# alibaba/TePDist

Hardware: AMD Instinct MI355X
Metric: tokens/sec (higher is better)
Workload: dtype bf16; 1 GPU; model=gpt2-345m, global_batch=64, seq_len=1024, parallelism=auto-planned-graph:dp1tp1pp1mesh[]micro1

## Files before the change

### tepdist_amd/ops/csrc/bindings.cpp

```cpp

#include <pybind11/pybind11.h>

#include <hip/hip_runtime.h>

#include <stdexcept>
#include <string>

#include "common.h"
#include "gemm_plan.h"
#include "kernels.h"

namespace py = pybind11;
using namespace tepdist;

namespace {

hipStream_t S(uintptr_t s) { return reinterpret_cast<hipStream_t>(s); }

void check_launch() { HIP_CHECK(hipGetLastError()); }

}

PYBIND11_MODULE(_tepdist_hip, m) {
  m.doc() = "TePDist-AMD gfx950 kernel library";

  m.def("gemm", [](uintptr_t A, uintptr_t B, uintptr_t C, uintptr_t Cpre,
                   uintptr_t bias, int M, int N, int K, int lda, int ldb,
                   int ldc, int64_t sa, int64_t sb, int64_t sc, int batch,
                   bool a_kc, bool b_kc, int epi, uintptr_t splitk_ws,
                   uintptr_t stream, uintptr_t colsum_out) {
    gemm_bf16(reinterpret_cast<void*>(A), reinterpret_cast<void*>(B),
              reinterpret_cast<void*>(C), reinterpret_cast<void*>(Cpre),
              reinterpret_cast<void*>(bias), M, N, K, lda, ldb, ldc, sa, sb,
              sc, batch, a_kc, b_kc, epi, reinterpret_cast<float*>(splitk_ws),
              reinterpret_cast<void*>(colsum_out), S(stream));
    check_launch();
  }, py::arg("A"), py::arg("B"), py::arg("C"), py::arg("Cpre"),
     py::arg("bias"), py::arg("M"), py::arg("N"), py::arg("K"),
     py::arg("lda"), py::arg("ldb"), py::arg("ldc"), py::arg("sa"),
     py::arg("sb"), py::arg("sc"), py::arg("batch"), py::arg("a_kc"),
     py::arg("b_kc"), py::arg("epi"), py::arg("splitk_ws"),
     py::arg("stream"), py::arg("colsum_out") = 0);

  m.def("gemm_ws_floats", [](int M, int N, int K, int lda, int ldb,
                             bool a_kc, bool b_kc, int epi, int batch,
                             bool colsum) {
    const GemmPlan p = gemm_plan(M, N, K, lda, ldb, a_kc, b_kc, epi, batch);
    if (colsum)
      if (const char* why = colsum_why_not(p, a_kc, b_kc, batch))
        throw std::runtime_error(std::string("gemm_ws_floats: ") + why);
    return gemm_ws_floats(p, M, N, colsum);
  }, py::arg("M"), py::arg("N"), py::arg("K"), py::arg("lda"),
     py::arg("ldb"), py::arg("a_kc") = true, py::arg("b_kc") = true,
     py::arg("epi") = 0, py::arg("batch") = 1, py::arg("colsum") = false);

  m.def("gemm_plan", [](int M, int N, int K, int lda, int ldb, bool a_kc,
                        bool b_kc, int epi, int batch) {
    const GemmPlan p = gemm_plan(M, N, K, lda, ldb, a_kc, b_kc, epi, batch);
    return py::make_tuple(p.kernel, p.split_k, p.k_chunk,
                          p.why_not ? p.why_not : "");
  }, py::arg("M"), py::arg("N"), py::arg("K"), py::arg("lda"),
     py::arg("ldb"), py::arg("a_kc") = true, py::arg("b_kc") = true,
     py::arg("epi") = 0, py::arg("batch") = 1);

  m.def("transpose", [](uintptr_t in, uintptr_t out, int R, int C,
                        int64_t si, int64_t so, int batch,
                        uintptr_t stream) {
    transpose_bf16(reinterpret_cast<void*>(in), reinterpret_cast<void*>(out),
                   R, C, si, so, batch, S(stream));
    check_launch();
  });

  m.def("layernorm_fwd", [](uintptr_t x, uintptr_t g, uintptr_t b, uintptr_t y,
                            uintptr_t mean, uintptr_t rstd, int rows, int cols,
                            float eps, uintptr_t stream, uintptr_t res,
                            uintptr_t sum_out) {
    layernorm_fwd_bf16(reinterpret_cast<void*>(x), reinterpret_cast<void*>(g),
                       reinterpret_cast<void*>(b), reinterpret_cast<void*>(y),
                       reinterpret_cast<float*>(mean),
                       reinterpret_cast<float*>(rstd), rows, cols, eps,
                       S(stream), reinterpret_cast<void*>(res),
                       reinterpret_cast<void*>(sum_out));
    check_launch();
  }, pybind11::arg("x"), pybind11::arg("g"), pybind11::arg("b"),
     pybind11::arg("y"), pybind11::arg("mean"), pybind11::arg("rstd"),
     pybind11::arg("rows"), pybind11::arg("cols"), pybind11::arg("eps"),
     pybind11::arg("stream"), pybind11::arg("res") = 0,
     pybind11::arg("sum_out") = 0);

  m.def("layernorm_bwd", [](uintptr_t dy, uintptr_t x, uintptr_t g,
                            uintptr_t mean, uintptr_t rstd, uintptr_t dx,
                            uintptr_t dg_part, uintptr_t db_part,
                            uintptr_t dgamma, uintptr_t dbeta, int rows,
                            int cols, int part_rows, uintptr_t stream,
                            uintptr_t dsum) {
    layernorm_bwd_bf16(reinterpret_cast<void*>(dy), reinterpret_cast<void*>(x),
                       reinterpret_cast<void*>(g),
                       reinterpret_cast<float*>(mean),
                       reinterpret_cast<float*>(rstd),
                       reinterpret_cast<void*>(dx),
                       reinterpret_cast<float*>(dg_part),
                       reinterpret_cast<float*>(db_part), rows, cols,
                       part_rows, S(stream), reinterpret_cast<void*>(dsum));
    check_launch();
    layernorm_bwd_reduce(reinterpret_cast<float*>(dg_part),
                         reinterpret_cast<float*>(db_part),
                         reinterpret_cast<void*>(dgamma),
                         reinterpret_cast<void*>(dbeta), part_rows, cols,
                         S(stream));
    check_launch();
  }, pybind11::arg("dy"), pybind11::arg("x"), pybind11::arg("g"),
     pybind11::arg("mean"), pybind11::arg("rstd"), pybind11::arg("dx"),
     pybind11::arg("dg_part"), pybind11::arg("db_part"),
     pybind11::arg("dgamma"), pybind11::arg("dbeta"), pybind11::arg("rows"),
     pybind11::arg("cols"), pybind11::arg("part_rows"),
     pybind11::arg("stream"), pybind11::arg("dsum") = 0);

  m.def("softmax_fwd", [](uintptr_t x, uintptr_t p, int64_t rows, int cols,
                          int sq, float scale, bool causal, uintptr_t stream) {
    softmax_fwd_bf16(reinterpret_cast<void*>(x), reinterpret_cast<void*>(p),
                     rows, cols, sq, scale, causal, S(stream));
    check_launch();
  });

  m.def("softmax_bwd", [](uintptr_t dp, uintptr_t p, uintptr_t ds,
                          int64_t rows, int cols, float scale,
                          uintptr_t stream) {
    softmax_bwd_bf16(reinterpret_cast<void*>(dp), reinterpret_cast<void*>(p),
                     reinterpret_cast<void*>(ds), rows, cols, scale,
                     S(stream));
    check_launch();
  });

  m.def("attention_fwd", [](uintptr_t q, uintptr_t k, uintptr_t v,
                            uintptr_t o, uintptr_t lse, int B, int H,
                            int seq, int D, float scale, bool causal,
                            int64_t q_bs, int64_t q_hs, int64_t q_rs,
                            int64_t o_bs, int64_t o_hs, int64_t o_rs,
                            uintptr_t stream) {
    attention_fwd_bf16(reinterpret_cast<void*>(q), reinterpret_cast<void*>(k),
                       reinterpret_cast<void*>(v), reinterpret_cast<void*>(o),
                       reinterpret_cast<float*>(lse), B, H, seq, D, scale,
                       causal, q_bs, q_hs, q_rs, o_bs, o_hs, o_rs, S(stream));
    check_launch();
  });

  m.def("attention_bwd", [](uintptr_t q, uintptr_t k, uintptr_t v,
                            uintptr_t o, uintptr_t dout, uintptr_t lse,
                            uintptr_t delta, uintptr_t dq, uintptr_t dk,
                            uintptr_t dv, int B, int H, int seq, int D,
                            float scale, bool causal, int64_t q_bs,
                            int64_t q_hs, int64_t q_rs, int64_t o_bs,
                            int64_t o_hs, int64_t o_rs, uintptr_t stream) {
    attention_bwd_bf16(
        reinterpret_cast<void*>(q), reinterpret_cast<void*>(k),
        reinterpret_cast<void*>(v), reinterpret_cast<void*>(o),
        reinterpret_cast<void*>(dout), reinterpret_cast<float*>(lse),
        reinterpret_cast<float*>(delta), reinterpret_cast<void*>(dq),
        reinterpret_cast<void*>(dk), reinterpret_cast<void*>(dv), B, H, seq,
        D, scale, causal, q_bs, q_hs, q_rs, o_bs, o_hs, o_rs, S(stream));
    check_launch();
  });

  m.def("decode_attention", [](uintptr_t q, uintptr_t k_new, uintptr_t v_new,
                               uintptr_t k_cache, uintptr_t v_cache,
                               uintptr_t pos, int pos_stride, uintptr_t out,
                               uintptr_t ws, int B, int H, int Hkv,
                               int S_max, int D, float scale, int splits,
                               bool rope, float rope_theta, int64_t q_bs,
                               int64_t q_hs, int64_t n_bs, int64_t n_hs,
                               int64_t c_bs, int64_t c_hs, int64_t c_rs,
                               uintptr_t stream) {
    decode_attention_bf16(
        reinterpret_cast<void*>(q), reinterpret_cast<void*>(k_new),
        reinterpret_cast<void*>(v_new), reinterpret_cast<void*>(k_cache),
        reinterpret_cast<void*>(v_cache),
        reinterpret_cast<const int64_t*>(pos), pos_stride,
        reinterpret_cast<void*>(out), reinterpret_cast<float*>(ws), B, H,
        Hkv, S_max, D, scale, splits, rope, rope_theta, q_bs, q_hs, n_bs,
        n_hs, c_bs, c_hs, c_rs, S(stream));
    check_launch();
  });

  m.def("moe_route_ws_ints", &moe_route_ws_ints);

  m.def("moe_route", [](uintptr_t gates, bool gates_fp32, uintptr_t topi,
                        uintptr_t slot, uintptr_t src, uintptr_t counts,
                        uintptr_t ws, int T, int E, int k, int C,
                        uintptr_t stream) {
    moe_route(reinterpret_cast<const void*>(gates), gates_fp32,
              reinterpret_cast<int*>(topi), reinterpret_cast<int*>(slot),
              reinterpret_cast<int*>(src), reinterpret_cast<int*>(counts),
              reinterpret_cast<int*>(ws), T, E, k, C, S(stream));
    check_launch();
  });

  m.def("moe_gather_rows", [](uintptr_t in, uintptr_t src, uintptr_t w,
                              uintptr_t out, int T, int k, int64_t EC, int d,
                              uintptr_t stream) {
    moe_gather_rows_bf16(reinterpret_cast<const void*>(in),
                         reinterpret_cast<const int*>(src),
                         reinterpret_cast<const float*>(w),
                         reinterpret_cast<void*>(out), T, k, EC, d,
                         S(stream));
    check_launch();
  });

  m.def("moe_reduce_rows", [](uintptr_t in, uintptr_t slot, uintptr_t w,
                              uintptr_t out, int T, int k, int64_t EC, int d,
                              uintptr_t stream) {
    moe_reduce_rows_bf16(reinterpret_cast<const void*>(in),
                         reinterpret_cast<const int*>(slot),
                         reinterpret_cast<const float*>(w),
                         reinterpret_cast<void*>(out), T, k, EC, d,
                         S(stream));
    check_launch();
  });

  m.def("moe_combine_dw", [](uintptr_t y, uintptr_t dout, uintptr_t slot,
                             uintptr_t dw, int T, int k, int64_t EC, int d,
                             uintptr_t stream) {
    moe_combine_dw_bf16(reinterpret_cast<const void*>(y),
                        reinterpret_cast<const void*>(dout),
                        reinterpret_cast<const int*>(slot),
                        reinterpret_cast<float*>(dw), T, k, EC, d, S(stream));
    check_launch();
  });

  m.def("embedding_fwd",[](uintptr_t ids, uintptr_t table, uintptr_t out,
                            int64_t n_ids, int dim, uintptr_t stream) {
    embedding_fwd_bf16(reinterpret_cast<const int64_t*>(ids),
                       reinterpret_cast<void*>(table),
                       reinterpret_cast<void*>(out), n_ids, dim, S(stream));
    check_launch();
  });

  m.def("embedding_bwd", [](uintptr_t dy, uintptr_t ids, uintptr_t grad_f32,
                            uintptr_t grad_bf16, int64_t n_ids, int vocab,
                            int dim, uintptr_t stream) {
    embedding_bwd_bf16(reinterpret_cast<void*>(dy),
                       reinterpret_cast<const int64_t*>(ids),
// ... 165 lines not shown
```

### tepdist_amd/ops/csrc/kernels.h

```cpp
#pragma once

#include <hip/hip_runtime.h>
#include <hip/hip_bf16.h>
#include <cstdint>

namespace tepdist {

using bf16 = __hip_bfloat16;

void gemm_bf16(const void* A, const void* B, void* C, void* c_pre,
               const void* bias, int M, int N, int K, int lda, int ldb,
               int ldc, int64_t stride_a, int64_t stride_b, int64_t stride_c,
               int batch, bool a_kc, bool b_kc, int epi, float* splitk_ws,
               void* colsum_out, hipStream_t stream);
void gemm256_bf16(const void* A, const void* B, void* C, void* c_pre,
                  const void* bias, int M, int N, int K, int lda, int ldb,
                  int ldc, int64_t stride_a, int64_t stride_b,
                  int64_t stride_c, int batch, bool k_outer, int epi,
                  int split_k, int k_chunk, float* colsum_parts,
                  hipStream_t stream);

void transpose_bf16(const void* in, void* out, int R, int C,
                    int64_t stride_in, int64_t stride_out, int batch,
                    hipStream_t stream);
void cast_ws_f32_bf16(const float* ws, void* db_out, int cols,
                      hipStream_t stream);
void transpose_dy_bf16(const void* dy, const void* pre, void* dy_t,
                       void* dy_nat, float* bias_ws, int R, int C,
                       hipStream_t stream);

void layernorm_fwd_bf16(const void* x, const void* gamma, const void* beta,
                        void* y, float* mean, float* rstd, int rows, int cols,
                        float eps, hipStream_t stream,
                        const void* res = nullptr, void* sum_out = nullptr);
void layernorm_bwd_bf16(const void* dy, const void* x, const void* gamma,
                        const float* mean, const float* rstd, void* dx,
                        float* dgamma_part, float* dbeta_part, int rows,
                        int cols, int part_rows, hipStream_t stream,
                        const void* dsum = nullptr);
void layernorm_bwd_reduce(const float* dgamma_part, const float* dbeta_part,
                          void* dgamma, void* dbeta, int part_rows, int cols,
                          hipStream_t stream);

void softmax_fwd_bf16(const void* x, void* p, int64_t rows, int cols, int sq,
                      float scale, bool causal, hipStream_t stream);
void softmax_bwd_bf16(const void* dp, const void* p, void* ds, int64_t rows,
                      int cols, float scale, hipStream_t stream);

void attention_fwd_bf16(const void* q, const void* k, const void* v, void* o,
                        float* lse, int B, int H, int S, int D, float scale,
                        bool causal, int64_t q_bs, int64_t q_hs, int64_t q_rs,
                        int64_t o_bs, int64_t o_hs, int64_t o_rs,
                        hipStream_t stream);
void attention_bwd_bf16(const void* q, const void* k, const void* v,
                        const void* o, const void* dout, const float* lse,
                        float* delta, void* dq, void* dk, void* dv,
                        int B, int H, int S, int D, float scale, bool causal,
                        int64_t q_bs, int64_t q_hs, int64_t q_rs,
                        int64_t o_bs, int64_t o_hs, int64_t o_rs,
                        hipStream_t stream);

void decode_attention_bf16(const void* q, const void* k_new,
                           const void* v_new, void* k_cache, void* v_cache,
                           const int64_t* pos, int pos_stride, void* out,
                           float* ws, int B, int H, int Hkv, int S_max,
                           int D, float scale, int splits, bool rope,
                           float rope_theta, int64_t q_bs,
                           int64_t q_hs, int64_t n_bs, int64_t n_hs,
                           int64_t c_bs, int64_t c_hs, int64_t c_rs,
                           hipStream_t stream);

int64_t moe_route_ws_ints(int T, int E);
void moe_route(const void* gates, bool gates_fp32, int* topi, int* slot,
               int* src, int* counts, int* ws, int T, int E, int k, int C,
               hipStream_t stream);
void moe_gather_rows_bf16(const void* in, const int* src, const float* w,
                          void* out, int T, int k, int64_t EC, int d,
                          hipStream_t stream);
void moe_reduce_rows_bf16(const void* in, const int* slot, const float* w,
                          void* out, int T, int k, int64_t EC, int d,
                          hipStream_t stream);
void moe_combine_dw_bf16(const void* y, const void* dout, const int* slot,
                         float* dw, int T, int k, int64_t EC, int d,
                         hipStream_t stream);

void embedding_fwd_bf16(const int64_t* ids, const void* table, void* out,
                        int64_t n_ids, int dim, hipStream_t stream);
void embedding_bwd_bf16(const void* dy, const int64_t* ids, float* grad_f32,
                        void* grad_bf16, int64_t n_ids, int vocab, int dim,
                        hipStream_t stream);

void cross_entropy_fwd_bf16(const void* logits, const int64_t* targets,
                            float* nll, float* lse, int64_t rows, int cols,
                            int ignore_index, hipStream_t stream);
void cross_entropy_bwd_bf16(const void* logits, const int64_t* targets,
                            const float* lse, const float* dscale,
                            void* dlogits, int64_t rows, int cols,
                            int ignore_index, hipStream_t stream);

void dropout_fwd_bf16(const void* x, void* y, uint8_t* mask, int64_t n,
                      float p, uint64_t seed, uint64_t offset,
                      hipStream_t stream);
void dropout_bwd_bf16(const void* dy, const uint8_t* mask, void* dx, int64_t n,
                      float p, hipStream_t stream);

void gelu_fwd_bf16(const void* x, void* y, int64_t n, hipStream_t stream);
void gelu_bwd_bf16(const void* dy, const void* x, void* dx, int64_t n,
                   hipStream_t stream);
void bias_sum_bf16(const void* dy, void* db, float* ws_zeroed, int64_t rows,
                   int cols, hipStream_t stream);

void adamw_bf16(void* param, float* master, const void* grad_bf16,
                const float* grad_f32, float* exp_avg, float* exp_avg_sq,
                int64_t n, float lr, float beta1, float beta2, float eps,
                float weight_decay, float bc1, float bc2, hipStream_t stream);

void adamw_mt_bf16(const int64_t* tabs, const int64_t* numel,
                   const float* wds, const unsigned char* ptypes,
                   const int* chunks, int nchunks, int nt,
                   float lr, float beta1, float beta2, float eps, float bc1,
                   float bc2, const float* hyper, hipStream_t stream);

void tr16_probe(float* out_pattern, float* out_uniform, hipStream_t stream);
void tr16_frag_probe(int* out, int C, hipStream_t stream);

void rmsnorm_fwd_bf16(const void* x, const void* g, void* y, float* rstd,
                      int64_t rows, int cols, float eps, hipStream_t stream);
void rmsnorm_bwd_bf16(const void* dy, const void* x, const void* g,
                      const float* rstd, void* dx, void* dgamma,
                      float* dg_part, int part_rows, int64_t rows, int cols,
                      hipStream_t stream);
void rope_bf16(const void* x, void* y, int64_t tokens, int heads, int D,
               int seq_len, float theta, bool backward, hipStream_t stream);
void swiglu_fwd_bf16(const void* a, const void* b, void* y, int64_t n,
                     hipStream_t stream);
void swiglu_bwd_bf16(const void* dy, const void* a, const void* b, void* da,
                     void* db, int64_t n, hipStream_t stream);

}
```

### tepdist_amd/ops/csrc/layernorm.hip

```cpp

#include <algorithm>
#include <stdexcept>

#include "common.h"
#include "kernels.h"

namespace tepdist {

namespace {

constexpr int NT = 256;

template <int NV, bool ADD = false>
__launch_bounds__(NT) __global__
void ln_fwd_kernel(const bf16_t* __restrict__ x, const bf16_t* __restrict__ g,
                   const bf16_t* __restrict__ b, bf16_t* __restrict__ y,
                   float* __restrict__ mean_out, float* __restrict__ rstd_out,
                   int rows, int cols, float eps,
                   const bf16_t* __restrict__ res = nullptr,
                   bf16_t* __restrict__ sum_out = nullptr) {
  const int lane = threadIdx.x & 63;
  const int wid = threadIdx.x >> 6;
  const int nwaves = gridDim.x * (NT / WAVE);

  for (int row = blockIdx.x * (NT / WAVE) + wid; row < rows; row += nwaves) {
    const bf16_t* xr = x + (int64_t)row * cols;
    const bf16_t* rr = ADD ? res + (int64_t)row * cols : nullptr;
    bf16_t* sr = ADD ? sum_out + (int64_t)row * cols : nullptr;
    float vals[NV * 8];
    float s = 0.f;
#pragma unroll
    for (int v = 0; v < NV; ++v) {
      const int c0 = v * WAVE * 8 + lane * 8;
      bf16x8 xv = {};
      bf16x8 rv = {};
      if (c0 + 8 <= cols) {
        xv = *reinterpret_cast<const bf16x8*>(xr + c0);
        if (ADD) rv = *reinterpret_cast<const bf16x8*>(rr + c0);
      } else {
#pragma unroll
        for (int e = 0; e < 8; ++e)
          if (c0 + e < cols) {
            xv[e] = xr[c0 + e];
            if (ADD) rv[e] = rr[c0 + e];
          }
      }
      bf16x8 sv;
#pragma unroll
      for (int e = 0; e < 8; ++e) {
        float f = bf2f(xv[e]);
        if (ADD) {
          sv[e] = f2bf(f + bf2f(rv[e]));
          f = bf2f(sv[e]);
        }
        vals[v * 8 + e] = f;
        s += f;
      }
      if (ADD && c0 < cols) {
        if (c0 + 8 <= cols) {
          *reinterpret_cast<bf16x8*>(sr + c0) = sv;
        } else {
          for (int e = 0; e < 8 && c0 + e < cols; ++e) sr[c0 + e] = sv[e];
        }
      }
    }
    s = wave_allreduce_sum(s);
    const float mean = s / cols;
    float ss = 0.f;
#pragma unroll
    for (int v = 0; v < NV; ++v)
#pragma unroll
      for (int e = 0; e < 8; ++e) {
        const int c = v * WAVE * 8 + lane * 8 + e;
        const float d = (c < cols) ? (vals[v * 8 + e] - mean) : 0.f;
        ss += d * d;
      }
    ss = wave_allreduce_sum(ss);
    const float rstd = rsqrtf(ss / cols + eps);
    if (lane == 0) {
      mean_out[row] = mean;
      rstd_out[row] = rstd;
    }
    bf16_t* yr = y + (int64_t)row * cols;
#pragma unroll
    for (int v = 0; v < NV; ++v) {
      const int c0 = v * WAVE * 8 + lane * 8;
      if (c0 >= cols) continue;
      bf16x8 yv = {};
      if (c0 + 8 <= cols) {
        const bf16x8 gv = *reinterpret_cast<const bf16x8*>(g + c0);
        const bf16x8 bv = *reinterpret_cast<const bf16x8*>(b + c0);
#pragma unroll
        for (int e = 0; e < 8; ++e) {
          const float xhat = (vals[v * 8 + e] - mean) * rstd;
          yv[e] = f2bf(xhat * bf2f(gv[e]) + bf2f(bv[e]));
        }
        *reinterpret_cast<bf16x8*>(yr + c0) = yv;
      } else {
        for (int e = 0; e < 8 && c0 + e < cols; ++e) {
          const float xhat = (vals[v * 8 + e] - mean) * rstd;
          yr[c0 + e] = f2bf(xhat * bf2f(g[c0 + e]) + bf2f(b[c0 + e]));
        }
      }
    }
  }
}

template <int NV, bool DS = false>
__launch_bounds__(NT) __global__
void ln_bwd_kernel(const bf16_t* __restrict__ dy, const bf16_t* __restrict__ x,
                   const bf16_t* __restrict__ g, const float* __restrict__ mean,
                   const float* __restrict__ rstd, bf16_t* __restrict__ dx,
                   float* __restrict__ dg_part, float* __restrict__ db_part,
                   int rows, int cols,
                   const bf16_t* __restrict__ dsum = nullptr) {
  const int lane = threadIdx.x & 63;
  const int wid = threadIdx.x >> 6;
  const int gwave = blockIdx.x * (NT / WAVE) + wid;
  const int nwaves = gridDim.x * (NT / WAVE);

  float dg_acc[NV * 8] = {};
  float db_acc[NV * 8] = {};

  bf16x8 gvv[NV];
#pragma unroll
  for (int v = 0; v < NV; ++v) {
    const int c0 = v * WAVE * 8 + lane * 8;
    bf16x8 gv = {};
    if (c0 + 8 <= cols) {
      gv = *reinterpret_cast<const bf16x8*>(g + c0);
    } else {
      for (int e = 0; e < 8 && c0 + e < cols; ++e) gv[e] = g[c0 + e];
    }
    gvv[v] = gv;
  }

  for (int row = gwave; row < rows; row += nwaves) {
    const bf16_t* dyr = dy + (int64_t)row * cols;
    const bf16_t* xr = x + (int64_t)row * cols;
    const float mu = mean[row], rs = rstd[row];
    float c1 = 0.f, c2 = 0.f;
    bf16x8 dyvv[NV], xvv[NV];
#pragma unroll
    for (int v = 0; v < NV; ++v) {
      const int c0 = v * WAVE * 8 + lane * 8;
      bf16x8 dyv = {}, xv = {};
      if (c0 + 8 <= cols) {
        dyv = *reinterpret_cast<const bf16x8*>(dyr + c0);
        xv = *reinterpret_cast<const bf16x8*>(xr + c0);
      } else {
        for (int e = 0; e < 8 && c0 + e < cols; ++e) {
          dyv[e] = dyr[c0 + e];
          xv[e] = xr[c0 + e];
        }
      }
      dyvv[v] = dyv;
      xvv[v] = xv;
#pragma unroll
      for (int e = 0; e < 8; ++e) {
        const int c = c0 + e;
        const float d = bf2f(dyv[e]);
        const float xhat = (c < cols) ? (bf2f(xv[e]) - mu) * rs : 0.f;
        const float gg = (c < cols) ? d * bf2f(gvv[v][e]) : 0.f;
        dg_acc[v * 8 + e] += d * xhat;
        db_acc[v * 8 + e] += d;
        c1 += gg;
        c2 += gg * xhat;
      }
    }
    c1 = wave_allreduce_sum(c1) / cols;
    c2 = wave_allreduce_sum(c2) / cols;
    bf16_t* dxr = dx + (int64_t)row * cols;
    const bf16_t* dsr = DS ? dsum + (int64_t)row * cols : nullptr;
#pragma unroll
    for (int v = 0; v < NV; ++v) {
      const int c0 = v * WAVE * 8 + lane * 8;
      if (c0 >= cols) continue;
      bf16x8 dsv = {};
      if (DS) {
        if (c0 + 8 <= cols) {
          dsv = *reinterpret_cast<const bf16x8*>(dsr + c0);
        } else {
          for (int e = 0; e < 8 && c0 + e < cols; ++e) dsv[e] = dsr[c0 + e];
        }
      }
      bf16x8 dxv;
#pragma unroll
      for (int e = 0; e < 8; ++e) {
        const float xhat = (bf2f(xvv[v][e]) - mu) * rs;
        const float gg = bf2f(dyvv[v][e]) * bf2f(gvv[v][e]);
        float d = (gg - c1 - xhat * c2) * rs;
        if (DS) d += bf2f(dsv[e]);
        dxv[e] = f2bf(d);
      }
      if (c0 + 8 <= cols) {
        *reinterpret_cast<bf16x8*>(dxr + c0) = dxv;
      } else {
        for (int e = 0; e < 8 && c0 + e < cols; ++e) dxr[c0 + e] = dxv[e];
      }
    }
  }

  float* dgp = dg_part + (int64_t)gwave * cols;
  float* dbp = db_part + (int64_t)gwave * cols;
#pragma unroll
  for (int v = 0; v < NV; ++v)
#pragma unroll
    for (int e = 0; e < 8; ++e) {
      const int c = v * WAVE * 8 + lane * 8 + e;
      if (c < cols) {
        dgp[c] = dg_acc[v * 8 + e];
        dbp[c] = db_acc[v * 8 + e];
      }
    }
}

__global__ void ln_bwd_reduce_kernel(const float* __restrict__ dg_part,
                                     const float* __restrict__ db_part,
                                     bf16_t* __restrict__ dgamma,
                                     bf16_t* __restrict__ dbeta,
                                     int part_rows, int cols) {
  const int lane = threadIdx.x & 63;
  const int c = blockIdx.x * (NT / WAVE) + (threadIdx.x >> 6);
  if (c >= cols) return;
  float sg = 0.f, sb = 0.f;
  for (int r = lane; r < part_rows; r += WAVE) {
    sg += dg_part[(int64_t)r * cols + c];
    sb += db_part[(int64_t)r * cols + c];
  }
  sg = wave_allreduce_sum(sg);
  sb = wave_allreduce_sum(sb);
  if (lane == 0) {
    dgamma[c] = f2bf(sg);
    dbeta[c] = f2bf(sb);
  }
}

int nv_for(int cols) { return (cols + WAVE * 8 - 1) / (WAVE * 8); }

}

void layernorm_fwd_bf16(const void* x, const void* gamma, const void* beta,
                        void* y, float* mean, float* rstd, int rows, int cols,
                        float eps, hipStream_t stream, const void* res,
                        void* sum_out) {
  const int blocks = std::min((rows + 3) / 4, 2048);
  const dim3 g(blocks), blk(NT);
  const bf16_t* xp = static_cast<const bf16_t*>(x);
  const bf16_t* gp = static_cast<const bf16_t*>(gamma);
  const bf16_t* bp = static_cast<const bf16_t*>(beta);
  bf16_t* yp = static_cast<bf16_t*>(y);
  const bf16_t* rp = static_cast<const bf16_t*>(res);
  bf16_t* sp = static_cast<bf16_t*>(sum_out);
#define LN_FWD(NV)                                                           \
  do {                                                                       \
    if (rp)                                                                  \
      hipLaunchKernelGGL((ln_fwd_kernel<NV, true>), g, blk, 0, stream, xp,  \
                         gp, bp, yp, mean, rstd, rows, cols, eps, rp, sp);  \
    else                                                                     \
      hipLaunchKernelGGL((ln_fwd_kernel<NV, false>), g, blk, 0, stream, xp, \
                         gp, bp, yp, mean, rstd, rows, cols, eps);          \
  } while (0)
  switch (nv_for(cols)) {
    case 1: LN_FWD(1); break;
    case 2: LN_FWD(2); break;
    case 3: LN_FWD(3); break;
    case 4: LN_FWD(4); break;
    case 5: LN_FWD(5); break;
    case 6: LN_FWD(6); break;
    default: throw std::runtime_error("layernorm: cols > 3072 unsupported");
  }
#undef LN_FWD
}

void layernorm_bwd_bf16(const void* dy, const void* x, const void* gamma,
                        const float* mean, const float* rstd, void* dx,
                        float* dgamma_part, float* dbeta_part, int rows,
                        int cols, int part_rows, hipStream_t stream,
                        const void* dsum) {
  const int blocks = part_rows / (NT / WAVE);
  const dim3 g(blocks), blk(NT);
  const bf16_t* dyp = static_cast<const bf16_t*>(dy);
  const bf16_t* xp = static_cast<const bf16_t*>(x);
  const bf16_t* gp = static_cast<const bf16_t*>(gamma);
  bf16_t* dxp = static_cast<bf16_t*>(dx);
  const bf16_t* dsp = static_cast<const bf16_t*>(dsum);
#define LN_BWD(NV)                                                           \
  do {                                                                       \
    if (dsp)                                                                 \
      hipLaunchKernelGGL((ln_bwd_kernel<NV, true>), g, blk, 0, stream, dyp, \
                         xp, gp, mean, rstd, dxp, dgamma_part, dbeta_part,  \
                         rows, cols, dsp);                                  \
    else                                                                     \
      hipLaunchKernelGGL((ln_bwd_kernel<NV, false>), g, blk, 0, stream,     \
                         dyp, xp, gp, mean, rstd, dxp, dgamma_part,         \
                         dbeta_part, rows, cols);                          \
  } while (0)
  switch (nv_for(cols)) {
    case 1: LN_BWD(1); break;
    case 2: LN_BWD(2); break;
    case 3: LN_BWD(3); break;
    case 4: LN_BWD(4); break;
    case 5: LN_BWD(5); break;
    case 6: LN_BWD(6); break;
    default: throw std::runtime_error("layernorm: cols > 3072 unsupported");
  }
#undef LN_BWD
}

void layernorm_bwd_reduce(const float* dgamma_part, const float* dbeta_part,
                          void* dgamma, void* dbeta, int part_rows, int cols,
                          hipStream_t stream) {
  hipLaunchKernelGGL(ln_bwd_reduce_kernel, dim3((cols + 3) / 4), dim3(NT),
                     0, stream, dgamma_part, dbeta_part,
                     static_cast<bf16_t*>(dgamma), static_cast<bf16_t*>(dbeta),
                     part_rows, cols);
}

}
```

### tepdist_amd/ops/hip.py

```python

from __future__ import annotations

import math
import os
from typing import Optional, Tuple

import torch

try:
    from tepdist_amd.ops import _tepdist_hip as ext
except ImportError as e:
    raise ImportError(
        "tepdist_amd HIP extension not built. Run "
        "`python tepdist_amd/ops/build_ext.py` (hipcc cross-compiles on a "
        "GPU-less box). No eager fallback is provided on GPU.") from e

BF16 = torch.bfloat16


def _stream() -> int:
    return torch.cuda.current_stream().cuda_stream


def _p(t: Optional[torch.Tensor]) -> int:
# ... 242 lines not shown
                  _stream())
    return out


def _wgrad_in_place(dyl: torch.Tensor, x: torch.Tensor) -> bool:
    (M, N), K = dyl.shape, x.shape[1]
    return dyl.stride(-1) == 1 and x.stride(-1) == 1 and ext.gemm_plan(
        N, K, M, dyl.stride(0), x.stride(0), False, False, 0, 1)[0] == 256


def wgrad(dyl: torch.Tensor, x: torch.Tensor, has_bias: bool):
    M, N = dyl.shape
    K = x.shape[1]
    def _db():
        return _bias_sum(dyl.contiguous()) if has_bias else None

    if not _wgrad_in_place(dyl, x):
        return matmul(dyl.t(), x), _db()

    def _hand():
        db = torch.empty(N, dtype=BF16, device=dyl.device) \
            if has_bias else None
        dw = _gemm_raw(dyl, x, False, False, N, K, M, dyl.stride(0),
                       x.stride(0), 0, 0, 1, colsum_out=db)[0]
        return dw, db

    def _lib():
        return torch.matmul(dyl.t(), x), _db()

    return _pick_backend(("lin_bw", M, N, K, has_bias), _hand, _lib)()


def linear_bwd(dy: torch.Tensor, x: torch.Tensor, w: torch.Tensor,
               has_bias: bool, act: str, pre_act: Optional[torch.Tensor]):
    dy = dy.contiguous()
    M, N = dy.shape
    K = w.shape[1]

    if _wgrad_in_place(dy, x):
        if act == "gelu":
            dyl = torch.empty_like(dy)
            ext.gelu_bwd(dy.data_ptr(), pre_act.data_ptr(), dyl.data_ptr(),
                         dy.numel(), _stream())
        else:
            dyl = dy

        def _dx_hip():
            wT = transpose2d(w)
            return _gemm_raw(dyl, wT, True, True, M, K, N, N, N, 0, 0, 1)[0]

        dx = _pick_backend(("lin_bx", M, N, K), _dx_hip,
                           lambda: torch.matmul(dyl, w))()
        dw, db = wgrad(dyl, x, has_bias)
        return dx, dw, db

    def _hip():
        dyl = dy
        wT = transpose2d(w)
        dyT = torch.empty(N, M, dtype=BF16, device=dy.device)
        if act == "gelu":
            dy_eff = torch.empty_like(dyl)
            ext.transpose_dy(dyl.data_ptr(), pre_act.data_ptr(),
                             dyT.data_ptr(), dy_eff.data_ptr(), 0, M, N,
                             _stream())
            dyl = dy_eff
        else:
            ext.transpose_dy(dyl.data_ptr(), 0, dyT.data_ptr(), 0, 0, M, N,
                             _stream())
        xT = transpose2d(x)
        dx, _ = _gemm_raw(dyl, wT, True, True, M, K, N, N, N, 0, 0, 1)
        dw, _ = _gemm_raw(dyT, xT, True, True, N, K, M, M, M, 0, 0, 1)
        return dx, dw, dyl

    def _blt():
        if act == "gelu":
            dyl = torch.empty_like(dy)
            ext.gelu_bwd(dy.data_ptr(), pre_act.data_ptr(), dyl.data_ptr(),
                         dy.numel(), _stream())
        else:
            dyl = dy
        dx = torch.matmul(dyl, w)
        dw = torch.matmul(dyl.t(), x)
        return dx, dw, dyl

    fn = _pick_backend(("lin_b", M, N, K, act), _hip, _blt)
    dx, dw, dy_eff = fn()
    db = None
    if has_bias:
        db = _bias_sum(dy_eff)
    return dx, dw, db


def matmul(a: torch.Tensor, b: torch.Tensor) -> torch.Tensor:
    key = ("mm", tuple(a.shape), tuple(b.shape),
           a.stride(-1) == 1, b.stride(-1) == 1)
    return _pick_backend(key, lambda: _matmul_hip(a, b),
                         lambda: torch.matmul(a, b))()


def _matmul_hip(a: torch.Tensor, b: torch.Tensor) -> torch.Tensor:
    assert a.dtype == BF16 and b.dtype == BF16
    squeeze = a.dim() == 2 and b.dim() == 2
    lead_shape = (a if a.dim() >= b.dim() else b).shape[:-2]
    if a.dim() == 2:
        a = a.unsqueeze(0)
    if b.dim() == 2:
        b = b.unsqueeze(0)
    if a.dim() > 3:
        a = a.reshape(-1, *a.shape[-2:]) if a.stride(-1) == 1 else \
            a.transpose(-1, -2).reshape(-1, a.shape[-1], a.shape[-2]).transpose(-1, -2)
    if b.dim() > 3:
        b = b.reshape(-1, *b.shape[-2:]) if b.stride(-1) == 1 else \
            b.transpose(-1, -2).reshape(-1, b.shape[-1], b.shape[-2]).transpose(-1, -2)
    M, K = a.shape[-2], a.shape[-1]
    K2, N = b.shape[-2], b.shape[-1]
    assert K == K2, (a.shape, b.shape)
    batch = max(a.shape[0], b.shape[0])

    def layout(t, contraction_is_last: bool):
        if t.stride(-1) == 1:
            inner_last = True
            ld = t.stride(-2)
        elif t.stride(-2) == 1:
            inner_last = False
            ld = t.stride(-1)
        else:
            t = t.contiguous()
            inner_last = True
            ld = t.stride(-2)
        kc = (inner_last == contraction_is_last)
        bs = t.stride(0) if t.shape[0] > 1 else 0
        return t, kc, ld, bs

    a, a_kc, lda, sa = layout(a, contraction_is_last=True)
    b, b_kc, ldb, sb = layout(b, contraction_is_last=False)
    if batch == 1 and M % 256 == 0 and N % 256 == 0 and K % 64 == 0 \
            and K >= 512 and not (
                not a_kc and not b_kc and ext.gemm_plan(
                    M, N, K, lda, ldb, False, False, 0, 1)[0] == 256):
        if not a_kc:
            a = transpose2d(a.reshape(K, M)).reshape(1, M, K)
            a_kc, lda = True, K
        if not b_kc:
            b = transpose2d(b.reshape(K, N)).reshape(1, N, K)
            b_kc, ldb = True, K
    c, _ = _gemm_raw(a, b, a_kc, b_kc, M, N, K, lda, ldb, sa, sb, batch,
                     device=a.device)
    if squeeze:
        return c.reshape(M, N)
    return c.reshape(*lead_shape, M, N)



LN_PART_ROWS = 1024


def layernorm_fwd(x: torch.Tensor, gamma: torch.Tensor, beta: torch.Tensor,
                  eps: float = 1e-5):
    x = x.contiguous()
    rows, cols = x.shape
    y = torch.empty_like(x)
    mean = torch.empty(rows, dtype=torch.float32, device=x.device)
    rstd = torch.empty(rows, dtype=torch.float32, device=x.device)
    ext.layernorm_fwd(x.data_ptr(), gamma.data_ptr(), beta.data_ptr(),
                      y.data_ptr(), mean.data_ptr(), rstd.data_ptr(), rows,
                      cols, eps, _stream())
    return y, mean, rstd


def layernorm_bwd(dy: torch.Tensor, x: torch.Tensor, gamma: torch.Tensor,
                  mean: torch.Tensor, rstd: torch.Tensor):
    dy = dy.contiguous()
    rows, cols = x.shape
    part = min(LN_PART_ROWS, max(4, (rows + 3) // 4 * 4))
    part = (part // 4) * 4
    dx = torch.empty_like(x)
    dg_part = torch.empty(part, cols, dtype=torch.float32, device=x.device)
    db_part = torch.empty(part, cols, dtype=torch.float32, device=x.device)
    dgamma = torch.empty_like(gamma)
    dbeta = torch.empty_like(gamma)
    ext.layernorm_bwd(dy.data_ptr(), x.data_ptr(), gamma.data_ptr(),
                      mean.data_ptr(), rstd.data_ptr(), dx.data_ptr(),
                      dg_part.data_ptr(), db_part.data_ptr(),
                      dgamma.data_ptr(), dbeta.data_ptr(), rows, cols, part,
                      _stream())
    return dx, dgamma, dbeta


def add_layernorm_fwd(x, res, gamma, beta, eps: float = 1e-5):
    x, res = x.contiguous(), res.contiguous()
    rows, cols = x.shape
    s = torch.empty_like(x)
    y = torch.empty_like(x)
    mean = torch.empty(rows, dtype=torch.float32, device=x.device)
    rstd = torch.empty(rows, dtype=torch.float32, device=x.device)
    ext.layernorm_fwd(x.data_ptr(), gamma.data_ptr(), beta.data_ptr(),
                      y.data_ptr(), mean.data_ptr(), rstd.data_ptr(), rows,
                      cols, eps, _stream(), res.data_ptr(), s.data_ptr())
    return s, y, mean, rstd


def add_layernorm_bwd(dy, dsum, s, gamma, mean, rstd):
    dy = dy.contiguous()
    dsum = dsum.contiguous() if dsum is not None else None
    rows, cols = s.shape
    part = min(LN_PART_ROWS, max(4, (rows + 3) // 4 * 4))
    part = (part // 4) * 4
    dx = torch.empty_like(s)
    dg_part = torch.empty(part, cols, dtype=torch.float32, device=s.device)
    db_part = torch.empty(part, cols, dtype=torch.float32, device=s.device)
    dgamma = torch.empty_like(gamma)
    dbeta = torch.empty_like(gamma)
    ext.layernorm_bwd(dy.data_ptr(), s.data_ptr(), gamma.data_ptr(),
                      mean.data_ptr(), rstd.data_ptr(), dx.data_ptr(),
                      dg_part.data_ptr(), db_part.data_ptr(),
                      dgamma.data_ptr(), dbeta.data_ptr(), rows, cols, part,
                      _stream(),
                      0 if dsum is None else dsum.data_ptr())
    return dx, dgamma, dbeta



def softmax_fwd(scores: torch.Tensor, scale: float = 1.0,
                causal: bool = False) -> torch.Tensor:
    scores = scores.contiguous()
    sq, sk = scores.shape[-2], scores.shape[-1]
    if causal and sq > sk:
        raise ValueError(f"causal softmax needs sq <= sk, got sq={sq} "
                         f"sk={sk}")
    rows = scores.numel() // sk
    p = torch.empty_like(scores)
    ext.softmax_fwd(scores.data_ptr(), p.data_ptr(), rows, sk, sq, scale,
                    causal, _stream())
    return p


def softmax_bwd(dp: torch.Tensor, p: torch.Tensor,
                scale: float = 1.0) -> torch.Tensor:
    dp = dp.contiguous()
    sk = p.shape[-1]
    rows = p.numel() // sk
    ds = torch.empty_like(p)
    ext.softmax_bwd(dp.data_ptr(), p.data_ptr(), ds.data_ptr(), rows, sk,
                    scale, _stream())
    return ds


_ATTN_IMPL = os.environ.get("TEPDIST_ATTN", "flash")


def _check_attention_operands(name: str, q: torch.Tensor, **others):
    if q.dim() != 4:
        raise ValueError(f"{name}: q must be [B, H, S, D], got "
                         f"{tuple(q.shape)}")
    for what, t in (("q", q),) + tuple(others.items()):
        if t.dtype != torch.bfloat16:
            raise ValueError(f"{name}: {what} is {t.dtype}, the flash "
                             "kernels are bf16-only")
        if t.shape != q.shape:
            raise ValueError(f"{name}: {what} is {tuple(t.shape)}, q is "
                             f"{tuple(q.shape)}")
        if t.device != q.device:
            raise ValueError(f"{name}: {what} is on {t.device}, q on "
                             f"{q.device}")


def _check_lse(name: str, lse: torch.Tensor, bh: int, S: int):
    if lse.dtype != torch.float32 or lse.numel() != bh * S:
        raise ValueError(f"{name}: lse must be fp32 with {bh} x {S} "
                         f"elements, got {lse.dtype} {tuple(lse.shape)}")
    return lse.contiguous()


def attention_fwd(q: torch.Tensor, k: torch.Tensor, v: torch.Tensor,
                  causal: bool = True):
    B, H, S, D = q.shape
    scale = 1.0 / math.sqrt(D)
    if _ATTN_IMPL == "composed" or D not in (64, 128):
        scores = matmul(q, k.transpose(-1, -2))
        p = softmax_fwd(scores, scale=scale, causal=causal)
        out = matmul(p, v)
        return out, (p,)
    _check_attention_operands("attention_fwd", q, k=k, v=v)
    q, k, v = q.contiguous(), k.contiguous(), v.contiguous()
    out = torch.empty_like(q)
    lse = torch.empty(B * H, S, dtype=torch.float32, device=q.device)
    sd = (H * S * D, S * D, D)
    ext.attention_fwd(q.data_ptr(), k.data_ptr(), v.data_ptr(),
                      out.data_ptr(), lse.data_ptr(), B, H, S, D, scale,
                      causal, *sd, *sd, _stream())
    return out, (out, lse)


def attention_bwd(dout: torch.Tensor, q, k, v, residuals,
                  causal: bool = True):
    B, H, S, D = q.shape
    scale = 1.0 / math.sqrt(D)
    if len(residuals) == 1:
        (p,) = residuals
        dv = matmul(p.transpose(-1, -2), dout)
        dp = matmul(dout, v.transpose(-1, -2))
        ds = softmax_bwd(dp, p, scale=scale)
        dq = matmul(ds, k)
        dk = matmul(ds.transpose(-1, -2), q)
        return dq, dk, dv
    out, lse = residuals
    _check_attention_operands("attention_bwd", q, k=k, v=v, out=out,
                              dout=dout)
    lse = _check_lse("attention_bwd", lse, B * H, S)
    q, k, v, out, dout = (t.contiguous() for t in (q, k, v, out, dout))
    delta = torch.empty(B * H, S, dtype=torch.float32, device=q.device)
    dq, dk, dv = (torch.empty(q.shape, dtype=q.dtype, device=q.device)
                  for _ in range(3))
    sd = (H * S * D, S * D, D)
    ext.attention_bwd(q.data_ptr(), k.data_ptr(), v.data_ptr(),
                      out.data_ptr(), dout.data_ptr(), lse.data_ptr(),
                      delta.data_ptr(), dq.data_ptr(), dk.data_ptr(),
                      dv.data_ptr(), B, H, S, D, scale, causal, *sd, *sd,
                      _stream())
    return dq, dk, dv


_DECODE_SPLITS = os.environ.get("TEPDIST_DECODE_SPLITS")


def decode_splits(bh: int, s_max: int, group: int = 1) -> int:
    if _DECODE_SPLITS:
        return max(1, min(32, int(_DECODE_SPLITS)))
    max_wg, min_rows = (256, 256) if group >= 4 else (64, 512)
    s = 1
    while s < 16 and bh * s * 2 <= max_wg and s_max // (s * 2) >= min_rows:
        s *= 2
    return s


def decode_attention(q: torch.Tensor, k_cache: torch.Tensor,
                     v_cache: torch.Tensor, positions: torch.Tensor,
                     k_new: Optional[torch.Tensor] = None,
                     v_new: Optional[torch.Tensor] = None,
                     scale: Optional[float] = None,
                     splits: Optional[int] = None,
                     rope_theta: Optional[float] = None) -> torch.Tensor:
    if q.dim() != 3 or k_cache.dim() != 4:
        raise ValueError("decode_attention: q [B,H,D], caches "
                         "[B,Hkv,S_max,D]")
    B, H, D = q.shape
    Hkv, S_max = k_cache.shape[1], k_cache.shape[2]
    if q.dtype != BF16 or k_cache.dtype != BF16 or v_cache.dtype != BF16:
        raise ValueError("decode_attention: hip backend is bf16-only")
    if D not in (64, 128):
        raise ValueError(f"decode_attention: head dim {D} not in (64, 128)")
    if (k_new is None) != (v_new is None):
        raise ValueError("decode_attention: k_new and v_new go together")
    if Hkv < 1 or H % Hkv != 0 or H // Hkv not in (1, 2, 4, 8):
        raise ValueError(f"decode_attention: {H} query heads over {Hkv} "
                         "K/V heads: the group size must be 1, 2, 4 or 8")
    if tuple(k_cache.shape) != (B, Hkv, S_max, D) or \
            v_cache.shape != k_cache.shape or \
            v_cache.stride() != k_cache.stride():
        raise ValueError("decode_attention: k_cache/v_cache must be "
# ... 451 lines not shown
```

Before: 353,200 tokens/s.

## Restructure layernorm backward with 8-wave blocks and in-block partial reduction

The layernorm backward kernel now runs 8 waves per block and reduces the per-wave dgamma/dbeta accumulators in shared memory, so each block writes one partial row instead of one per wave. This cuts the partial buffer and the work of the final reduce. The dsum load moves up with the dy and x loads, and a no-tail template variant drops the bounds checks. The reduce kernel now spreads rows across 16 waves per column tile. In exchange the kernel uses more shared memory and adds two block-wide syncs, and the compiler barriers (empty asm) constrain instruction scheduling.

```diff
diff --git a/tepdist_amd/ops/csrc/bindings.cpp b/tepdist_amd/ops/csrc/bindings.cpp
--- a/tepdist_amd/ops/csrc/bindings.cpp
+++ b/tepdist_amd/ops/csrc/bindings.cpp
@@ -87,6 +87,8 @@
      pybind11::arg("rows"), pybind11::arg("cols"), pybind11::arg("eps"),
      pybind11::arg("stream"), pybind11::arg("res") = 0,
      pybind11::arg("sum_out") = 0);
+
+  m.attr("LN_BWD_BLOCK_WAVES") = layernorm_bwd_block_waves();
 
   m.def("layernorm_bwd", [](uintptr_t dy, uintptr_t x, uintptr_t g,
                             uintptr_t mean, uintptr_t rstd, uintptr_t dx,
diff --git a/tepdist_amd/ops/csrc/kernels.h b/tepdist_amd/ops/csrc/kernels.h
--- a/tepdist_amd/ops/csrc/kernels.h
+++ b/tepdist_amd/ops/csrc/kernels.h
@@ -33,6 +33,7 @@
                         void* y, float* mean, float* rstd, int rows, int cols,
                         float eps, hipStream_t stream,
                         const void* res = nullptr, void* sum_out = nullptr);
+int layernorm_bwd_block_waves();
 void layernorm_bwd_bf16(const void* dy, const void* x, const void* gamma,
                         const float* mean, const float* rstd, void* dx,
                         float* dgamma_part, float* dbeta_part, int rows,
diff --git a/tepdist_amd/ops/csrc/layernorm.hip b/tepdist_amd/ops/csrc/layernorm.hip
--- a/tepdist_amd/ops/csrc/layernorm.hip
+++ b/tepdist_amd/ops/csrc/layernorm.hip
@@ -106,18 +106,163 @@
   }
 }
 
-template <int NV, bool DS = false>
-__launch_bounds__(NT) __global__
+constexpr int BWD_WAVES = 8;
+constexpr int BWD_NT = BWD_WAVES * WAVE;
+
+template <int NV, bool DS>
+struct LnBwdRow {
+  bf16x8 dy[NV], x[NV], ds[DS ? NV : 1];
+  float mu, rs;
+};
+
+template <int NV, bool DS, bool TAIL>
+DEV_INLINE void ln_bwd_load_row(LnBwdRow<NV, DS>& r,
+                                const bf16_t* __restrict__ dy,
+                                const bf16_t* __restrict__ x,
+                                const bf16_t* __restrict__ dsum,
+                                const float* __restrict__ mean,
+                                const float* __restrict__ rstd, int row,
+                                int cols, int lane) {
+  const bf16_t* dyr = dy + (int64_t)row * cols;
+  const bf16_t* xr = x + (int64_t)row * cols;
+  const bf16_t* dsr = DS ? dsum + (int64_t)row * cols : nullptr;
+  r.mu = mean[row];
+  r.rs = rstd[row];
+#pragma unroll
+  for (int v = 0; v < NV; ++v) {
+    const int c0 = v * WAVE * 8 + lane * 8;
+    bf16x8 dyv = {}, xv = {}, dsv = {};
+    if (!TAIL) {
+      const int cl = c0 < cols ? c0 : 0;
+      dyv = *reinterpret_cast<const bf16x8*>(dyr + cl);
+      xv = *reinterpret_cast<const bf16x8*>(xr + cl);
+      if (DS) dsv = *reinterpret_cast<const bf16x8*>(dsr + cl);
+    } else if (c0 + 8 <= cols) {
+      dyv = *reinterpret_cast<const bf16x8*>(dyr + c0);
+      xv = *reinterpret_cast<const bf16x8*>(xr + c0);
+      if (DS) dsv = *reinterpret_cast<const bf16x8*>(dsr + c0);
+    } else {
+      for (int e = 0; e < 8 && c0 + e < cols; ++e) {
+        dyv[e] = dyr[c0 + e];
+        xv[e] = xr[c0 + e];
+        if (DS) dsv[e] = dsr[c0 + e];
+      }
+    }
+    r.dy[v] = dyv;
+    r.x[v] = xv;
+    if (DS) r.ds[v] = dsv;
+  }
+}
+
+DEV_INLINE void ln_bwd_reload(bf16x8& v, float after) {
+  u32x4 t = __builtin_bit_cast(u32x4, v);
+  asm volatile("" : "+v"(t) : "v"(after));
+  v = __builtin_bit_cast(bf16x8, t);
+}
+
+DEV_INLINE void ln_bwd_tie(bf16x8& a, bf16x8& b) {
+  u32x4 ta = __builtin_bit_cast(u32x4, a), tb = __builtin_bit_cast(u32x4, b);
+  asm volatile("" : "+v"(ta), "+v"(tb));
+  a = __builtin_bit_cast(bf16x8, ta);
+  b = __builtin_bit_cast(bf16x8, tb);
+}
+
+template <int NV>
+DEV_INLINE void ln_bwd_block_sum(const float (&acc)[NV * 8], float* red,
+                                 float* __restrict__ part_row, int cols) {
+  constexpr int PITCH = NV * WAVE * 8;
+  const int lane = threadIdx.x & 63;
+  const int wid = threadIdx.x >> 6;
+#pragma unroll
+  for (int v = 0; v < NV; ++v) {
+    float* p = red + wid * PITCH + v * WAVE * 8 + lane * 8;
+    *reinterpret_cast<f32x4*>(p) = f32x4{acc[v * 8 + 0], acc[v * 8 + 1],
+                                          acc[v * 8 + 2], acc[v * 8 + 3]};
+    *reinterpret_cast<f32x4*>(p + 4) = f32x4{acc[v * 8 + 4], acc[v * 8 + 5],
+                                              acc[v * 8 + 6], acc[v * 8 + 7]};
+  }
+  __syncthreads();
+#pragma unroll
+  for (int c = threadIdx.x; c < PITCH; c += BWD_NT) {
+    float s = 0.f;
+#pragma unroll
+    for (int w = 0; w < BWD_WAVES; ++w) s += red[w * PITCH + c];
+    if (c < cols) part_row[c] = s;
+  }
+  __syncthreads();
+}
+
+template <int NV, bool DS, bool TAIL>
+DEV_INLINE void ln_bwd_row(LnBwdRow<NV, DS>& r, const bf16x8 (&gvv)[NV],
+                           float (&dg_acc)[NV * 8], float (&db_acc)[NV * 8],
+                           bf16_t* __restrict__ dx, int row, int cols,
+                           int lane) {
+  const float mu = r.mu, rs = r.rs;
+  float c1 = 0.f, c2 = 0.f;
+  if (DS) {
+#pragma unroll
+    for (int v = 0; v < NV; ++v) ln_bwd_tie(r.ds[v], r.dy[v]);
+  }
+#pragma unroll
+  for (int v = 0; v < NV; ++v) {
+    const int c0 = v * WAVE * 8 + lane * 8;
+#pragma unroll
+    for (int e = 0; e < 8; ++e) {
+#pragma clang fp contract(off)
+      const int c = c0 + e;
+      const float d = bf2f(r.dy[v][e]);
+      const float xhat = (c < cols) ? (bf2f(r.x[v][e]) - mu) * rs : 0.f;
+      const float gg = (c < cols) ? d * bf2f(gvv[v][e]) : 0.f;
+      dg_acc[v * 8 + e] = __builtin_fmaf(d, xhat, dg_acc[v * 8 + e]);
+      db_acc[v * 8 + e] += d;
+      c1 += gg;
+      c2 = NV == 1 ? __builtin_fmaf(gg, xhat, c2) : c2 + gg * xhat;
+    }
+  }
+#pragma unroll
+  for (int i = 0; i < NV * 8; ++i)
+    asm volatile("" : "+v"(dg_acc[i]), "+v"(db_acc[i]));
+  c1 = wave_allreduce_sum(c1) / cols;
+  c2 = wave_allreduce_sum(c2) / cols;
+#pragma unroll
+  for (int v = 0; v < NV; ++v) {
+    ln_bwd_reload(r.x[v], c2);
+    ln_bwd_reload(r.dy[v], c2);
+  }
+  bf16_t* dxr = dx + (int64_t)row * cols;
+#pragma unroll
+  for (int v = 0; v < NV; ++v) {
+    const int c0 = v * WAVE * 8 + lane * 8;
+    if (c0 >= cols) continue;
+    bf16x8 dxv;
+#pragma unroll
+    for (int e = 0; e < 8; ++e) {
+#pragma clang fp contract(off)
+      const float xhat = (bf2f(r.x[v][e]) - mu) * rs;
+      const float gg = bf2f(r.dy[v][e]) * bf2f(gvv[v][e]);
+      const float u = __builtin_fmaf(-xhat, c2, gg - c1);
+      const float d = DS ? __builtin_fmaf(u, rs, bf2f(r.ds[v][e])) : u * rs;
+      dxv[e] = f2bf(d);
+    }
+    if (!TAIL || c0 + 8 <= cols) {
+      *reinterpret_cast<bf16x8*>(dxr + c0) = dxv;
+    } else {
+      for (int e = 0; e < 8 && c0 + e < cols; ++e) dxr[c0 + e] = dxv[e];
+    }
+  }
+}
+
+template <int NV, bool DS, bool TAIL>
+__launch_bounds__(BWD_NT, (!TAIL && NV <= 2) ? 4 : 2) __global__
 void ln_bwd_kernel(const bf16_t* __restrict__ dy, const bf16_t* __restrict__ x,
                    const bf16_t* __restrict__ g, const float* __restrict__ mean,
                    const float* __restrict__ rstd, bf16_t* __restrict__ dx,
                    float* __restrict__ dg_part, float* __restrict__ db_part,
-                   int rows, int cols,
-                   const bf16_t* __restrict__ dsum = nullptr) {
+                   int rows, int cols, const bf16_t* __restrict__ dsum) {
+  __shared__ __attribute__((aligned(16))) float red[BWD_WAVES * NV * WAVE * 8];
   const int lane = threadIdx.x & 63;
   const int wid = threadIdx.x >> 6;
-  const int gwave = blockIdx.x * (NT / WAVE) + wid;
-  const int nwaves = gridDim.x * (NT / WAVE);
+  const int nwaves = gridDim.x * BWD_WAVES;
 
   float dg_acc[NV * 8] = {};
   float db_acc[NV * 8] = {};
@@ -135,102 +280,48 @@
     gvv[v] = gv;
   }
 
-  for (int row = gwave; row < rows; row += nwaves) {
-    const bf16_t* dyr = dy + (int64_t)row * cols;
-    const bf16_t* xr = x + (int64_t)row * cols;
-    const float mu = mean[row], rs = rstd[row];
-    float c1 = 0.f, c2 = 0.f;
-    bf16x8 dyvv[NV], xvv[NV];
-#pragma unroll
-    for (int v = 0; v < NV; ++v) {
-      const int c0 = v * WAVE * 8 + lane * 8;
-      bf16x8 dyv = {}, xv = {};
-      if (c0 + 8 <= cols) {
-        dyv = *reinterpret_cast<const bf16x8*>(dyr + c0);
-        xv = *reinterpret_cast<const bf16x8*>(xr + c0);
-      } else {
-        for (int e = 0; e < 8 && c0 + e < cols; ++e) {
-          dyv[e] = dyr[c0 + e];
-          xv[e] = xr[c0 + e];
-        }
-      }
-      dyvv[v] = dyv;
-      xvv[v] = xv;
-#pragma unroll
-      for (int e = 0; e < 8; ++e) {
-        const int c = c0 + e;
-        const float d = bf2f(dyv[e]);
-        const float xhat = (c < cols) ? (bf2f(xv[e]) - mu) * rs : 0.f;
-        const float gg = (c < cols) ? d * bf2f(gvv[v][e]) : 0.f;
-        dg_acc[v * 8 + e] += d * xhat;
-        db_acc[v * 8 + e] += d;
-        c1 += gg;
-        c2 += gg * xhat;
-      }
-    }
-    c1 = wave_allreduce_sum(c1) / cols;
-    c2 = wave_allreduce_sum(c2) / cols;
-    bf16_t* dxr = dx + (int64_t)row * cols;
-    const bf16_t* dsr = DS ? dsum + (int64_t)row * cols : nullptr;
-#pragma unroll
-    for (int v = 0; v < NV; ++v) {
-      const int c0 = v * WAVE * 8 + lane * 8;
-      if (c0 >= cols) continue;
-      bf16x8 dsv = {};
-      if (DS) {
-        if (c0 + 8 <= cols) {
-          dsv = *reinterpret_cast<const bf16x8*>(dsr + c0);
-        } else {
-          for (int e = 0; e < 8 && c0 + e < cols; ++e) dsv[e] = dsr[c0 + e];
-        }
-      }
-      bf16x8 dxv;
-#pragma unroll
-      for (int e = 0; e < 8; ++e) {
-        const float xhat = (bf2f(xvv[v][e]) - mu) * rs;
-        const float gg = bf2f(dyvv[v][e]) * bf2f(gvv[v][e]);
-        float d = (gg - c1 - xhat * c2) * rs;
-        if (DS) d += bf2f(dsv[e]);
-        dxv[e] = f2bf(d);
-      }
-      if (c0 + 8 <= cols) {
-        *reinterpret_cast<bf16x8*>(dxr + c0) = dxv;
-      } else {
-        for (int e = 0; e < 8 && c0 + e < cols; ++e) dxr[c0 + e] = dxv[e];
-      }
-    }
-  }
-
-  float* dgp = dg_part + (int64_t)gwave * cols;
-  float* dbp = db_part + (int64_t)gwave * cols;
-#pragma unroll
-  for (int v = 0; v < NV; ++v)
-#pragma unroll
-    for (int e = 0; e < 8; ++e) {
-      const int c = v * WAVE * 8 + lane * 8 + e;
-      if (c < cols) {
-        dgp[c] = dg_acc[v * 8 + e];
-        dbp[c] = db_acc[v * 8 + e];
-      }
-    }
-}
-
-__global__ void ln_bwd_reduce_kernel(const float* __restrict__ dg_part,
-                                     const float* __restrict__ db_part,
-                                     bf16_t* __restrict__ dgamma,
-                                     bf16_t* __restrict__ dbeta,
-                                     int part_rows, int cols) {
+  LnBwdRow<NV, DS> r;
+  for (int row = blockIdx.x * BWD_WAVES + wid; row < rows; row += nwaves) {
+    ln_bwd_load_row<NV, DS, TAIL>(r, dy, x, dsum, mean, rstd, row, cols, lane);
+    ln_bwd_row<NV, DS, TAIL>(r, gvv, dg_acc, db_acc, dx, row, cols, lane);
+  }
+
+  ln_bwd_block_sum<NV>(dg_acc, red, dg_part + (int64_t)blockIdx.x * cols,
+                       cols);
+  ln_bwd_block_sum<NV>(db_acc, red, db_part + (int64_t)blockIdx.x * cols,
+                       cols);
+}
+
+constexpr int RED_WAVES = 16;
+
+__launch_bounds__(RED_WAVES * WAVE) __global__
+void ln_bwd_reduce_kernel(const float* __restrict__ dg_part,
+                          const float* __restrict__ db_part,
+                          bf16_t* __restrict__ dgamma,
+                          bf16_t* __restrict__ dbeta, int part_rows,
+                          int cols) {
+  __shared__ float sg_s[RED_WAVES][WAVE], sb_s[RED_WAVES][WAVE];
   const int lane = threadIdx.x & 63;
-  const int c = blockIdx.x * (NT / WAVE) + (threadIdx.x >> 6);
-  if (c >= cols) return;
+  const int wid = threadIdx.x >> 6;
+  const int c = blockIdx.x * WAVE + lane;
   float sg = 0.f, sb = 0.f;
-  for (int r = lane; r < part_rows; r += WAVE) {
-    sg += dg_part[(int64_t)r * cols + c];
-    sb += db_part[(int64_t)r * cols + c];
-  }
-  sg = wave_allreduce_sum(sg);
-  sb = wave_allreduce_sum(sb);
-  if (lane == 0) {
+  if (c < cols) {
+    for (int r = wid; r < part_rows; r += RED_WAVES) {
+      sg += dg_part[(int64_t)r * cols + c];
+      sb += db_part[(int64_t)r * cols + c];
+    }
+  }
+  sg_s[wid][lane] = sg;
+  sb_s[wid][lane] = sb;
+  __syncthreads();
+  if (wid == 0 && c < cols) {
+    sg = 0.f;
+    sb = 0.f;
+#pragma unroll
+    for (int w = 0; w < RED_WAVES; ++w) {
+      sg += sg_s[w][lane];
+      sb += sb_s[w][lane];
+    }
     dgamma[c] = f2bf(sg);
     dbeta[c] = f2bf(sb);
   }
@@ -273,28 +364,32 @@
 #undef LN_FWD
 }
 
+int layernorm_bwd_block_waves() { return BWD_WAVES; }
+
 void layernorm_bwd_bf16(const void* dy, const void* x, const void* gamma,
                         const float* mean, const float* rstd, void* dx,
                         float* dgamma_part, float* dbeta_part, int rows,
                         int cols, int part_rows, hipStream_t stream,
                         const void* dsum) {
-  const int blocks = part_rows / (NT / WAVE);
-  const dim3 g(blocks), blk(NT);
+  if (part_rows < 1)
+    throw std::runtime_error("layernorm_bwd: needs at least one partial row");
+  const dim3 g(part_rows), blk(BWD_NT);
   const bf16_t* dyp = static_cast<const bf16_t*>(dy);
   const bf16_t* xp = static_cast<const bf16_t*>(x);
   const bf16_t* gp = static_cast<const bf16_t*>(gamma);
   bf16_t* dxp = static_cast<bf16_t*>(dx);
   const bf16_t* dsp = static_cast<const bf16_t*>(dsum);
+#define LN_BWD_K(NV, DS, TAIL)                                              \
+  hipLaunchKernelGGL((ln_bwd_kernel<NV, DS, TAIL>), g, blk, 0, stream, dyp, \
+                     xp, gp, mean, rstd, dxp, dgamma_part, dbeta_part,      \
+                     rows, cols, dsp)
 #define LN_BWD(NV)                                                           \
   do {                                                                       \
-    if (dsp)                                                                 \
-      hipLaunchKernelGGL((ln_bwd_kernel<NV, true>), g, blk, 0, stream, dyp, \
-                         xp, gp, mean, rstd, dxp, dgamma_part, dbeta_part,  \
-                         rows, cols, dsp);                                  \
-    else                                                                     \
-      hipLaunchKernelGGL((ln_bwd_kernel<NV, false>), g, blk, 0, stream,     \
-                         dyp, xp, gp, mean, rstd, dxp, dgamma_part,         \
-                         dbeta_part, rows, cols);                          \
+    if (cols % 8) {                                                          \
+      if (dsp) LN_BWD_K(NV, true, true); else LN_BWD_K(NV, false, true);    \
+    } else {                                                                 \
+      if (dsp) LN_BWD_K(NV, true, false); else LN_BWD_K(NV, false, false);  \
+    }                                                                        \
   } while (0)
   switch (nv_for(cols)) {
     case 1: LN_BWD(1); break;
@@ -306,15 +401,16 @@
     default: throw std::runtime_error("layernorm: cols > 3072 unsupported");
   }
 #undef LN_BWD
+#undef LN_BWD_K
 }
 
 void layernorm_bwd_reduce(const float* dgamma_part, const float* dbeta_part,
                           void* dgamma, void* dbeta, int part_rows, int cols,
                           hipStream_t stream) {
-  hipLaunchKernelGGL(ln_bwd_reduce_kernel, dim3((cols + 3) / 4), dim3(NT),
-                     0, stream, dgamma_part, dbeta_part,
-                     static_cast<bf16_t*>(dgamma), static_cast<bf16_t*>(dbeta),
-                     part_rows, cols);
-}
-
-}
+  hipLaunchKernelGGL(ln_bwd_reduce_kernel, dim3((cols + WAVE - 1) / WAVE),
+                     dim3(RED_WAVES * WAVE), 0, stream, dgamma_part,
+                     dbeta_part, static_cast<bf16_t*>(dgamma),
+                     static_cast<bf16_t*>(dbeta), part_rows, cols);
+}
+
+}
diff --git a/tepdist_amd/ops/hip.py b/tepdist_amd/ops/hip.py
--- a/tepdist_amd/ops/hip.py
+++ b/tepdist_amd/ops/hip.py
@@ -418,7 +418,13 @@
 
 
 
-LN_PART_ROWS = 1024
+LN_BWD_BLOCK_WAVES = ext.LN_BWD_BLOCK_WAVES
+LN_PART_ROWS = 512
+LN_BWD_WAVES = LN_PART_ROWS * LN_BWD_BLOCK_WAVES
+
+
+def _ln_bwd_blocks(rows: int) -> int:
+    return min(LN_PART_ROWS, max(1, -(-rows // LN_BWD_BLOCK_WAVES)))
 
 
 def layernorm_fwd(x: torch.Tensor, gamma: torch.Tensor, beta: torch.Tensor,
@@ -438,8 +444,7 @@
                   mean: torch.Tensor, rstd: torch.Tensor):
     dy = dy.contiguous()
     rows, cols = x.shape
-    part = min(LN_PART_ROWS, max(4, (rows + 3) // 4 * 4))
-    part = (part // 4) * 4
+    part = _ln_bwd_blocks(rows)
     dx = torch.empty_like(x)
     dg_part = torch.empty(part, cols, dtype=torch.float32, device=x.device)
     db_part = torch.empty(part, cols, dtype=torch.float32, device=x.device)
@@ -470,8 +475,7 @@
     dy = dy.contiguous()
     dsum = dsum.contiguous() if dsum is not None else None
     rows, cols = s.shape
-    part = min(LN_PART_ROWS, max(4, (rows + 3) // 4 * 4))
-    part = (part // 4) * 4
+    part = _ln_bwd_blocks(rows)
     dx = torch.empty_like(s)
     dg_part = torch.empty(part, cols, dtype=torch.float32, device=s.device)
     db_part = torch.empty(part, cols, dtype=torch.float32, device=s.device)
```

New measurement: 358,100 tokens/s (median of 6 runs). +1.4%, better.
